# SenseTime-FVG/OpenDWM

Measured on NVIDIA H100. Metric: CTSD-3.5 6view x 16f denoise-steps/sec, higher is better.
Workload: dtype fp16

## Files before the change

### opendwm_b200/csrc/common.cuh

```cuda
#pragma once

#include <cuda.h>
#include <cuda_runtime.h>
#include <cuda_bf16.h>
#include <cuda_fp16.h>
#include <cuda_fp8.h>
#include <stdint.h>
#include <stdio.h>

namespace dwm {

void set_last_error(const char* fmt, ...);

#define DWM_CHECK_CUDA(expr)                                                   \
  do {                                                                         \
    cudaError_t _e = (expr);                                                   \
    if (_e != cudaSuccess) {                                                   \
      ::dwm::set_last_error("%s failed: %s (%s:%d)", #expr,                    \
                            cudaGetErrorString(_e), __FILE__, __LINE__);       \
      return -2;                                                               \
    }                                                                          \
  } while (0)

#define DWM_REQUIRE(cond, ...)                                                 \
  do {                                                                         \
    if (!(cond)) {                                                             \
      ::dwm::set_last_error(__VA_ARGS__);                                      \
      return -1;                                                               \
    }                                                                          \
  } while (0)

int make_tmap_2d(CUtensorMap* map, const void* base, uint64_t rows, uint64_t cols,
                 uint64_t ld, uint32_t box_rows, uint32_t box_cols, int elem_bytes);

int make_tmap_3d(CUtensorMap* map, const void* base, uint64_t items, uint64_t rows, uint64_t cols,
                 uint64_t ld, uint64_t item_ld, uint32_t box_rows, uint32_t box_cols, int elem_bytes);

int make_tmap_nd(CUtensorMap* map, const void* base, int rank, const uint64_t* dims,
                 const uint64_t* strides_bytes, const uint32_t* box, int elem_bytes);

int sm_count();

inline bool is_aligned(const void* p, uintptr_t bytes) { return (reinterpret_cast<uintptr_t>(p) & (bytes - 1)) == 0; }

#ifdef __CUDACC__
__device__ __forceinline__ uint32_t smem_u32(const void* p) {
  return static_cast<uint32_t>(__cvta_generic_to_shared(p));
}

__device__ __forceinline__ bool elect_one() {
  uint32_t pred = 0;
  asm volatile(
      "{\n\t"
      ".reg .pred P;\n\t"
      "elect.sync _|P, 0xffffffff;\n\t"
      "selp.u32 %0, 1, 0, P;\n\t"
      "}\n"
      : "=r"(pred));
  return pred != 0;
}

__device__ __forceinline__ void mbar_init(uint64_t* bar, uint32_t count) {
  asm volatile("mbarrier.init.shared::cta.b64 [%0], %1;" ::"r"(smem_u32(bar)), "r"(count));
}
__device__ __forceinline__ void fence_barrier_init() {
  asm volatile("fence.mbarrier_init.release.cluster;" ::: "memory");
}
__device__ __forceinline__ void fence_proxy_async() {
  asm volatile("fence.proxy.async.shared::cta;" ::: "memory");
}
__device__ __forceinline__ void mbar_expect_tx(uint64_t* bar, uint32_t bytes) {
  asm volatile("mbarrier.arrive.expect_tx.shared::cta.b64 _, [%0], %1;" ::"r"(smem_u32(bar)),
               "r"(bytes)
               : "memory");
}
__device__ __forceinline__ void mbar_arrive(uint64_t* bar) {
  asm volatile("mbarrier.arrive.shared::cta.b64 _, [%0];" ::"r"(smem_u32(bar)) : "memory");
}
__device__ __forceinline__ bool mbar_try_wait(uint64_t* bar, uint32_t parity) {
  uint32_t ok;
  asm volatile(
      "{\n\t"
      ".reg .pred P;\n\t"
      "mbarrier.try_wait.parity.shared::cta.b64 P, [%1], %2;\n\t"
      "selp.u32 %0, 1, 0, P;\n\t"
      "}\n"
      : "=r"(ok)
      : "r"(smem_u32(bar)), "r"(parity)
      : "memory");
  return ok != 0;
}
__device__ __forceinline__ void mbar_wait(uint64_t* bar, uint32_t parity) {
#ifdef DWM_BOUNDED_WAIT
  for (uint32_t it = 0; it < (1u << 26); ++it) {
    if (mbar_try_wait(bar, parity)) return;
  }
  printf("dwm_b200: mbarrier wait timed out (block %d thread %d)\n", blockIdx.x, threadIdx.x);
  __trap();
#else
  while (!mbar_try_wait(bar, parity)) {
  }
#endif
}

__device__ __forceinline__ void tma_prefetch_desc(const CUtensorMap* m) {
  asm volatile("prefetch.tensormap [%0];" ::"l"(reinterpret_cast<uint64_t>(m)) : "memory");
}
__device__ __forceinline__ void tma_load_2d(const CUtensorMap* m, uint64_t* bar, void* smem,
                                            int32_t c0, int32_t c1, uint64_t cache_hint) {
  asm volatile(
      "cp.async.bulk.tensor.2d.shared::cluster.global.mbarrier::complete_tx::bytes.L2::cache_hint"
      " [%0], [%1, {%3, %4}], [%2], %5;"
      :
      : "r"(smem_u32(smem)), "l"(reinterpret_cast<uint64_t>(m)), "r"(smem_u32(bar)), "r"(c0),
        "r"(c1), "l"(cache_hint)
      : "memory");
}
constexpr uint64_t kEvictNormal = 0x1000000000000000ull;
constexpr uint64_t kEvictFirst = 0x12F0000000000000ull;
constexpr uint64_t kEvictLast = 0x14F0000000000000ull;
__device__ __forceinline__ void tma_prefetch_2d(const CUtensorMap* m, int32_t c0, int32_t c1) {
  asm volatile("cp.async.bulk.prefetch.tensor.2d.L2.global.tile [%0, {%1, %2}];" ::"l"(
                   reinterpret_cast<uint64_t>(m)),
               "r"(c0), "r"(c1)
               : "memory");
}
__device__ __forceinline__ void tma_prefetch_5d(const CUtensorMap* m, int c0, int c1, int c2, int c3, int c4) {
  asm volatile("cp.async.bulk.prefetch.tensor.5d.L2.global.tile [%0, {%1, %2, %3, %4, %5}];" ::"l"(
                   reinterpret_cast<uint64_t>(m)),
               "r"(c0), "r"(c1), "r"(c2), "r"(c3), "r"(c4)
               : "memory");
}
__device__ __forceinline__ void tma_load_5d(const CUtensorMap* m, uint64_t* bar, void* smem, int c0,
                                            int c1, int c2, int c3, int c4, uint64_t hint) {
  asm volatile(
      "cp.async.bulk.tensor.5d.shared::cluster.global.mbarrier::complete_tx::bytes.L2::cache_hint"
      " [%0], [%1, {%3, %4, %5, %6, %7}], [%2], %8;"
      :
      : "r"(smem_u32(smem)), "l"(reinterpret_cast<uint64_t>(m)), "r"(smem_u32(bar)), "r"(c0), "r"(c1),
        "r"(c2), "r"(c3), "r"(c4), "l"(hint)
      : "memory");
}

__device__ __forceinline__ void tma_store_3d(const CUtensorMap* m, const void* smem, int c0, int c1, int c2) {
  asm volatile("cp.async.bulk.tensor.3d.global.shared::cta.bulk_group [%0, {%2, %3, %4}], [%1];" ::"l"(
                   reinterpret_cast<uint64_t>(m)),
               "r"(smem_u32(smem)), "r"(c0), "r"(c1), "r"(c2)
               : "memory");
}
__device__ __forceinline__ void bulk_commit() { asm volatile("cp.async.bulk.commit_group;" ::: "memory"); }
__device__ __forceinline__ void bulk_wait_read_all() { asm volatile("cp.async.bulk.wait_group.read 0;" ::: "memory"); }
__device__ __forceinline__ void bulk_wait_all() { asm volatile("cp.async.bulk.wait_group 0;" ::: "memory"); }
__device__ __forceinline__ void named_bar_sync(int id, int n) {
  asm volatile("bar.sync %0, %1;" ::"r"(id), "r"(n) : "memory");
}
__device__ __forceinline__ void stmatrix_x4(uint32_t addr, uint32_t r0, uint32_t r1, uint32_t r2, uint32_t r3) {
  asm volatile("stmatrix.sync.aligned.m8n8.x4.shared.b16 [%0], {%1, %2, %3, %4};" ::"r"(addr), "r"(r0), "r"(r1),
               "r"(r2), "r"(r3)
               : "memory");
}

__device__ __forceinline__ uint32_t cluster_ctarank() {
  uint32_t r;
  asm volatile("mov.u32 %0, %%cluster_ctarank;" : "=r"(r));
  return r;
}
__device__ __forceinline__ void cluster_sync_all() {
  asm volatile("barrier.cluster.arrive.release.aligned;" ::: "memory");
  asm volatile("barrier.cluster.wait.acquire.aligned;" ::: "memory");
}
__device__ __forceinline__ uint32_t mapa_u32(uint32_t smem_addr, uint32_t rank) {
  uint32_t r;
  asm volatile("mapa.shared::cluster.u32 %0, %1, %2;" : "=r"(r) : "r"(smem_addr), "r"(rank));
  return r;
}
__device__ __forceinline__ void mbar_arrive_remote(uint32_t cluster_addr) {
  asm volatile("mbarrier.arrive.shared::cluster.b64 _, [%0];" ::"r"(cluster_addr) : "memory");
}
__device__ __forceinline__ void tma_load_2d_mc(const CUtensorMap* m, uint64_t* bar, void* smem, int32_t c0,
                                               int32_t c1, uint16_t mask, uint64_t cache_hint) {
  asm volatile(
      "cp.async.bulk.tensor.2d.shared::cluster.global.mbarrier::complete_tx::bytes.multicast::cluster"
      ".L2::cache_hint [%0], [%1, {%3, %4}], [%2], %5, %6;"
      :
      : "r"(smem_u32(smem)), "l"(reinterpret_cast<uint64_t>(m)), "r"(smem_u32(bar)), "r"(c0), "r"(c1),
        "h"(mask), "l"(cache_hint)
      : "memory");
}

__device__ __forceinline__ uint64_t gmma_desc_sw128(uint32_t smem_addr) {
  uint64_t d = 0;
  d |= static_cast<uint64_t>((smem_addr & 0x3FFFF) >> 4);
  d |= static_cast<uint64_t>(1) << 16;
  d |= static_cast<uint64_t>(1024 >> 4) << 32;
  d |= static_cast<uint64_t>(1) << 62;
  return d;
}
__device__ __forceinline__ void wgmma_fence() { asm volatile("wgmma.fence.sync.aligned;" ::: "memory"); }
__device__ __forceinline__ void wgmma_commit() { asm volatile("wgmma.commit_group.sync.aligned;" ::: "memory"); }
template <int N>
__device__ __forceinline__ void wgmma_wait() {
  asm volatile("wgmma.wait_group.sync.aligned %0;" ::"n"(N) : "memory");
}
template <int N>
__device__ __forceinline__ void fence_operands(float (&d)[N]) {
#pragma unroll
  for (int i = 0; i < N; ++i) asm volatile("" : "+f"(d[i])::"memory");
}
template <int R>
__device__ __forceinline__ void setmaxnreg_inc() { asm volatile("setmaxnreg.inc.sync.aligned.u32 %0;" ::"n"(R)); }
template <int R>
__device__ __forceinline__ void setmaxnreg_dec() { asm volatile("setmaxnreg.dec.sync.aligned.u32 %0;" ::"n"(R)); }

__device__ __forceinline__ float gelu_erf(float x) {
  return 0.5f * x * (1.0f + erff(x * 0.70710678118654752440f));
}
__device__ __forceinline__ float gelu_tanh(float x) {
  const float k2 = 2.0f * 0.7978845608028654f;
  const float u2 = k2 * (x + 0.044715f * x * x * x);
  return __fdividef(x, 1.0f + __expf(-u2));
}
__device__ __forceinline__ float silu(float x) { return x / (1.0f + __expf(-x)); }

template <typename T>
struct Cvt;
template <>
struct Cvt<__nv_bfloat16> {
  __device__ static __forceinline__ uint32_t pack2(float a, float b) {
    __nv_bfloat162 v = __floats2bfloat162_rn(a, b);
    return *reinterpret_cast<uint32_t*>(&v);
  }
  __device__ static __forceinline__ float2 unpack2(uint32_t u) {
    __nv_bfloat162 v = *reinterpret_cast<__nv_bfloat162*>(&u);
    return __bfloat1622float2(v);
  }
  __device__ static __forceinline__ float to_f(__nv_bfloat16 v) { return __bfloat162float(v); }
  __device__ static __forceinline__ __nv_bfloat16 from_f(float v) { return __float2bfloat16_rn(v); }
};
template <>
struct Cvt<__half> {
  __device__ static __forceinline__ uint32_t pack2(float a, float b) {
    __half2 v = __floats2half2_rn(a, b);
    return *reinterpret_cast<uint32_t*>(&v);
  }
  __device__ static __forceinline__ float2 unpack2(uint32_t u) {
    __half2 v = *reinterpret_cast<__half2*>(&u);
    return __half22float2(v);
  }
  __device__ static __forceinline__ float to_f(__half v) { return __half2float(v); }
  __device__ static __forceinline__ __half from_f(float v) { return __float2half_rn(v); }
};

__device__ __forceinline__ float warp_sum(float v) {
#pragma unroll
  for (int o = 16; o > 0; o >>= 1) v += __shfl_xor_sync(0xffffffffu, v, o);
  return v;
}
__device__ __forceinline__ float warp_max(float v) {
#pragma unroll
  for (int o = 16; o > 0; o >>= 1) v = fmaxf(v, __shfl_xor_sync(0xffffffffu, v, o));
  return v;
}

constexpr float kE4M3Max = 448.f;
__device__ __forceinline__ float e4m3_inv(float amax) { return amax > 0.f ? __fdiv_rn(kE4M3Max, amax) : 0.f; }
__device__ __forceinline__ float e4m3_scale(float amax) { return amax > 0.f ? __fdiv_rn(amax, kE4M3Max) : 1.f; }
__device__ __forceinline__ uint32_t e4m3x4(float a, float b, float c, float d, float inv) {
  uint16_t lo, hi;
  asm("cvt.rn.satfinite.e4m3x2.f32 %0, %1, %2;" : "=h"(lo) : "f"(__fmul_rn(b, inv)), "f"(__fmul_rn(a, inv)));
  asm("cvt.rn.satfinite.e4m3x2.f32 %0, %1, %2;" : "=h"(hi) : "f"(__fmul_rn(d, inv)), "f"(__fmul_rn(c, inv)));
  return static_cast<uint32_t>(lo) | (static_cast<uint32_t>(hi) << 16);
}
#endif

}
```

### opendwm_b200/csrc/gemm.cu

```cuda
#include <stdlib.h>
#include <string.h>

#include "gemm_epilogue.cuh"

namespace dwm {

constexpr int STAGES = 4;
constexpr int A_STAGE_BYTES = BM * BK * 2;

static_assert(EPI_BOXES_BYTES >= EPI_STAGE_BYTES, "epilogue region");
template <int NT>
struct GemmCfg {
  static constexpr int kBStageBytes = NT * BK * 2;
  static constexpr int kSmemBytes =
      STAGES * (A_STAGE_BYTES + kBStageBytes) + EPI_BOXES_BYTES + 1024  + 256 ;
};

template <typename TA, typename T, int EPI, int NT, int CL>
__global__ void __launch_bounds__(GEMM_THREADS, 1)
    gemm_wgmma_kernel(const __grid_constant__ CUtensorMap tmap_a,
                      const __grid_constant__ CUtensorMap tmap_b,
                      const __grid_constant__ CUtensorMap tmap_out, int M, int N, int K,
                      EpiParams p) {
  constexpr int B_STAGE_BYTES = GemmCfg<NT>::kBStageBytes;
  constexpr int BKE = BK * 2 / static_cast<int>(sizeof(TA));
  extern __shared__ uint8_t smem_raw[];
  uint8_t* smem = smem_raw + ((1024u - (smem_u32(smem_raw) & 1023u)) & 1023u);
  uint8_t* smem_a = smem;
  uint8_t* smem_b = smem + STAGES * A_STAGE_BYTES;
  uint8_t* epi_region = smem + STAGES * (A_STAGE_BYTES + B_STAGE_BYTES);
  float* epi_stage = reinterpret_cast<float*>(epi_region);
  uint64_t* bars = reinterpret_cast<uint64_t*>(epi_region + EPI_BOXES_BYTES);
  uint64_t* full_bar = bars;
  uint64_t* empty_bar = bars + STAGES;

  const int warp = threadIdx.x >> 5;
  const int lane = threadIdx.x & 31;
  const int wg = threadIdx.x >> 7;
  const uint32_t rank = CL == 2 ? cluster_ctarank() : 0u;

  const int m_blocks = (M + BM - 1) / BM;
  const int n_blocks = (N + NT - 1) / NT;
  const int k_blocks = (K + BKE - 1) / BKE;
  const int num_tiles = ((m_blocks + CL - 1) / CL) * n_blocks;
  const int first = static_cast<int>(blockIdx.x) / CL, step = static_cast<int>(gridDim.x) / CL;

  if (warp == 0 && lane == 0) {
    tma_prefetch_desc(&tmap_a);
    tma_prefetch_desc(&tmap_b);
    for (int s = 0; s < STAGES; ++s) {
      mbar_init(&full_bar[s], 1);
      mbar_init(&empty_bar[s], CL * EPI_WARPS);
    }
    fence_barrier_init();
  }
  if constexpr (CL == 2) cluster_sync_all(); else __syncthreads();

  if (wg == 0) {
    setmaxnreg_dec<PRODUCER_REGS>();
    if (warp == 0 && elect_one()) {
      int stage = 0;
      uint32_t phase = 0;
      for (int tile = first; tile < num_tiles; tile += step) {
        const int m_blk = (tile / n_blocks) * CL + static_cast<int>(rank);
        const int n_blk = tile % n_blocks;
        for (int kb = 0; kb < k_blocks; ++kb) {
          mbar_wait(&empty_bar[stage], phase ^ 1);
          mbar_expect_tx(&full_bar[stage], A_STAGE_BYTES + B_STAGE_BYTES);
          tma_load_2d(&tmap_a, &full_bar[stage], smem_a + stage * A_STAGE_BYTES, kb * BKE,
                      m_blk * BM, kEvictNormal);
          if constexpr (CL == 2) {
            tma_load_2d_mc(&tmap_b, &full_bar[stage], smem_b + stage * B_STAGE_BYTES + rank * (B_STAGE_BYTES / 2),
                           kb * BKE, n_blk * NT + static_cast<int>(rank) * (NT / 2), 0x3, kEvictLast);
          } else {
            tma_load_2d(&tmap_b, &full_bar[stage], smem_b + stage * B_STAGE_BYTES, kb * BKE,
                        n_blk * NT, kEvictLast);
          }
          if (++stage == STAGES) {
            stage = 0;
            phase ^= 1;
          }
        }
      }
    }
    __syncwarp();
  } else {
    setmaxnreg_inc<CONSUMER_REGS>();
    const int cw = wg - 1;
    const int wrow = cw * 64 + (warp & 3) * 16;
    float* stg = epi_stage + (warp - 4) * 512;
    TmaOut tout{epi_out16(EPI) && p.tma_out, &tmap_out, epi_region + cw * 2 * EPI_BOX_BYTES, 1 + cw,
                (threadIdx.x & 127) == 0, 0};
    int stage = 0;
    uint32_t phase = 0;
    for (int tile = first; tile < num_tiles; tile += step) {
      const int m_blk = (tile / n_blocks) * CL + static_cast<int>(rank);
      const int n_blk = tile % n_blocks;
      const int t = threadIdx.x & 127;
      prefetch_resid_tile<EPI, NT>(p, m_blk * BM + cw * 64 + (t >> 1), M, n_blk * NT, N, t & 1);
      float acc[NT / 2];
      wg_mainloop<TA, NT, CL>(acc, smem_a, A_STAGE_BYTES, cw * 64 * 128, smem_b, B_STAGE_BYTES, full_bar,
                              empty_bar, STAGES, k_blocks, stage, phase, lane, rank ^ 1u);
      if constexpr (sizeof(TA) == 1)
        dequant_frag<NT>(acc, p.a_scale, p.w_scale, m_blk * BM + wrow, M, n_blk * NT, N, lane);
      drain_tile<T, EPI, NT>(acc, stg, m_blk * BM, wrow, M, n_blk * NT, N, p, lane, TileGeom{0, 0, 0, 0, 0}, &tout);
    }
    if (tout.on && tout.leader) bulk_wait_all();
  }
  if constexpr (CL == 2) cluster_sync_all();
}

int g_resid_tma = 1;

template <typename TA, typename T, int EPI, int NT, int CL>
static int launch_gemm(const dwm_linear_args* a, cudaStream_t stream) {
  constexpr int eb = static_cast<int>(sizeof(TA));
  CUtensorMap ta, tb;
  int rc = make_tmap_2d(&ta, a->A, a->M, a->K, a->lda, BM, BK * 2 / eb, eb);
  if (rc) return rc;
  rc = make_tmap_2d(&tb, a->W, a->N, a->K, a->ldw, NT / CL, BK * 2 / eb, eb);
  if (rc) return rc;

  EpiParams p;
  fill_epi_params(p, a);
  p.resid_prefetch = g_resid_tma;
  CUtensorMap to = {};
  if (epi_out16(EPI) && a->n_peer_out == 0) {
    const long long rpi = a->rows_per_item > 0 ? a->rows_per_item : a->M;
    const long long items = a->M / rpi;
    const long long item_ld = (a->rows_per_item > 0 ? a->out_item_stride : a->M) * a->ldo;
    const long long n_out = (EPI == DWM_EPI_GEGLU || EPI == DWM_EPI_GEGLU_TANH) ? a->N / 2 : a->N;
    if (items > 0) {
      rc = make_tmap_3d(&to, reinterpret_cast<const T*>(a->out) + a->out_row_offset * a->ldo, items, rpi, n_out,
                        a->ldo, item_ld, 64, 64, 2);
      if (rc) return rc;
    }
    p.tma_out = 1;
    p.out_rpi = static_cast<int>(rpi);
    p.out_items = static_cast<int>(items);
  }

  constexpr int smem_bytes = GemmCfg<NT>::kSmemBytes;
  auto kern = gemm_wgmma_kernel<TA, T, EPI, NT, CL>;
  static bool attr_set = false;
  if (!attr_set) {
    DWM_CHECK_CUDA(cudaFuncSetAttribute(kern, cudaFuncAttributeMaxDynamicSharedMemorySize, smem_bytes));
    attr_set = true;
  }
  const long long m_blocks = (a->M + BM - 1) / BM;
  const long long n_blocks = (a->N + NT - 1) / NT;
  const long long tiles = ((m_blocks + CL - 1) / CL) * n_blocks;
  const long long slots = sm_count() / CL;
  const int grid = CL * static_cast<int>(tiles < slots ? tiles : slots);
  const int Mi = static_cast<int>(a->M), Ni = static_cast<int>(a->N), Ki = static_cast<int>(a->K);
  if constexpr (CL == 1) {
    kern<<<grid, GEMM_THREADS, smem_bytes, stream>>>(ta, tb, to, Mi, Ni, Ki, p);
  } else {
    DWM_CHECK_CUDA(launch_cluster2(kern, grid, GEMM_THREADS, smem_bytes, stream,
                                   ta, tb, to, Mi, Ni, Ki, p));
  }
  DWM_CHECK_CUDA(cudaGetLastError());
  return 0;
}

int g_gemm_bn = 0;
int g_gemm_2cta = -1;

static int pick_tile_n(const dwm_linear_args* a, int cl) {
  if (a->epilogue == DWM_EPI_GEGLU || a->epilogue == DWM_EPI_GEGLU_TANH) return 256;
  if (g_gemm_bn == 128 || g_gemm_bn == 256) return g_gemm_bn;
  const long long slots = sm_count() / cl;
  const long long m_groups = ((a->M + BM - 1) / BM + cl - 1) / cl;
  const long long t256 = m_groups * ((a->N + 255) / 256), t128 = m_groups * ((a->N + 127) / 128);
  const long long waves256 = (t256 + slots - 1) / slots, waves128 = (t128 + slots - 1) / slots;
  return waves128 * 128 * 10 < waves256 * 256 * 9 ? 128 : 256;
}

template <typename TA, typename T, int EPI, int CL>
static int launch_pick_n(const dwm_linear_args* a, cudaStream_t s) {
  if (pick_tile_n(a, CL) == 128) return launch_gemm<TA, T, EPI, 128, CL>(a, s);
  return launch_gemm<TA, T, EPI, 256, CL>(a, s);
}

template <typename TA, typename T, int CL, typename TF = T>
static int dispatch_epi(const dwm_linear_args* a, cudaStream_t s) {
  if constexpr (sizeof(TA) == 2) {
    if (a->epilogue == DWM_EPI_STORE && a->act == DWM_ACT_QUICK_GELU)
      return launch_pick_n<TA, T, EPI_STORE_QUICK_GELU, CL>(a, s);
    if (a->epilogue == DWM_EPI_GEGLU_TANH) return launch_gemm<TA, T, DWM_EPI_GEGLU_TANH, 256, CL>(a, s);
  }
  switch (a->epilogue) {
    case DWM_EPI_STORE: return launch_pick_n<TA, T, DWM_EPI_STORE, CL>(a, s);
    case DWM_EPI_GEGLU: return launch_gemm<TA, T, DWM_EPI_GEGLU, 256, CL>(a, s);
    case DWM_EPI_QKNORM: return launch_pick_n<TA, T, DWM_EPI_QKNORM, CL>(a, s);
    case DWM_EPI_RESID: return launch_pick_n<TA, TF, DWM_EPI_RESID, CL>(a, s);
    case DWM_EPI_F32: return launch_pick_n<TA, TF, DWM_EPI_F32, CL>(a, s);
    default: set_last_error("dwm_b200_linear: unknown epilogue %d", a->epilogue); return -1;
  }
}

template <int CL>
static int dispatch_e4m3(const dwm_linear_args* a, cudaStream_t s) {
  if (a->out_dtype == DWM_BF16) return dispatch_epi<__nv_fp8_e4m3, __nv_bfloat16, CL>(a, s);
  return dispatch_epi<__nv_fp8_e4m3, __half, CL, __nv_bfloat16>(a, s);
}

}

namespace dwm { int g_attn_tc = -1; extern int g_ln_staged; extern int g_conv_2cta; extern int g_conv_halo; }

extern "C" int dwm_b200_set_option(const char* name, int value) {
  using namespace dwm;
  DWM_REQUIRE(name != nullptr, "dwm_b200_set_option: null name");
  if (strcmp(name, "attn_tc") == 0) { g_attn_tc = value; return 0; }
  if (strcmp(name, "ln_staged") == 0) { g_ln_staged = value; return 0; }
  if (strcmp(name, "gemm_bn") == 0) { g_gemm_bn = value; return 0; }
  if (strcmp(name, "gemm_2cta") == 0) { g_gemm_2cta = value; return 0; }
  if (strcmp(name, "resid_tma") == 0) { g_resid_tma = value; return 0; }
  if (strcmp(name, "conv_2cta") == 0) { g_conv_2cta = value; return 0; }
  if (strcmp(name, "conv_halo") == 0) { g_conv_halo = value; return 0; }
  set_last_error("dwm_b200_set_option: unknown option %s", name);
  return -1;
}

extern "C" int dwm_b200_linear(const dwm_linear_args* a, dwm_stream_t stream) {
  using namespace dwm;
  DWM_REQUIRE(a != nullptr, "dwm_b200_linear: null args");
  DWM_REQUIRE(a->M > 0 && a->N > 0 && a->K > 0, "dwm_b200_linear: empty problem %lld x %lld x %lld",
              (long long)a->M, (long long)a->N, (long long)a->K);
  DWM_REQUIRE(a->M < (1ll << 31) && a->N < (1ll << 31) && a->K < (1ll << 31),
              "dwm_b200_linear: dimension exceeds int32");
  DWM_REQUIRE(a->A && a->W && a->out, "dwm_b200_linear: null A/W/out");
  DWM_REQUIRE(a->K % 8 == 0 && a->lda % 8 == 0 && a->ldw % 8 == 0,
              "dwm_b200_linear: K, lda, ldw must be multiples of 8 (16-byte TMA pitch); got %lld %lld %lld",
              (long long)a->K, (long long)a->lda, (long long)a->ldw);
  if (a->dtype == DWM_E4M3) {
    DWM_REQUIRE(a->K % 16 == 0 && a->lda % 16 == 0 && a->ldw % 16 == 0,
                "dwm_b200_linear: E4M3 needs K, lda, ldw multiples of 16 (16-byte TMA pitch); got %lld %lld %lld",
                (long long)a->K, (long long)a->lda, (long long)a->ldw);
    DWM_REQUIRE(a->a_scale && a->w_scale, "dwm_b200_linear: E4M3 operands need a_scale and w_scale");
    DWM_REQUIRE(a->out_dtype == DWM_BF16 || a->out_dtype == DWM_F16,
                "dwm_b200_linear: E4M3 operands need out_dtype DWM_BF16 or DWM_F16, got %d", a->out_dtype);
    DWM_REQUIRE((reinterpret_cast<uintptr_t>(a->w_scale) & 7) == 0,
                "dwm_b200_linear: w_scale must be 8-byte aligned");
  }
  DWM_REQUIRE((reinterpret_cast<uintptr_t>(a->A) & 15) == 0 &&
                  (reinterpret_cast<uintptr_t>(a->W) & 15) == 0 &&
                  (reinterpret_cast<uintptr_t>(a->out) & 15) == 0,
              "dwm_b200_linear: A, W, out must be 16-byte aligned");
  DWM_REQUIRE(a->N % 32 == 0, "dwm_b200_linear: N must be a multiple of 32, got %lld", (long long)a->N);
  DWM_REQUIRE(a->ldo % 8 == 0, "dwm_b200_linear: ldo must be a multiple of 8");
  if (a->epilogue == DWM_EPI_GEGLU || a->epilogue == DWM_EPI_GEGLU_TANH)
    DWM_REQUIRE(a->N % 256 == 0, "dwm_b200_linear: GEGLU needs N %% 256 == 0 (packed weight)");
  if (a->epilogue == DWM_EPI_GEGLU_TANH || a->act == DWM_ACT_QUICK_GELU) {
    DWM_REQUIRE(a->dtype == DWM_BF16 || a->dtype == DWM_F16,
                "dwm_b200_linear: DWM_EPI_GEGLU_TANH and DWM_ACT_QUICK_GELU need 16-bit operands");
    DWM_REQUIRE(a->act != DWM_ACT_QUICK_GELU || a->epilogue == DWM_EPI_STORE,
                "dwm_b200_linear: DWM_ACT_QUICK_GELU needs the DWM_EPI_STORE epilogue");
  }
  if (a->epilogue == DWM_EPI_QKNORM) {
    DWM_REQUIRE(a->N % 64 == 0 && a->qk_region > 0 && a->qk_region % 64 == 0 && a->q_norm_weight &&
                    (a->k_norm_weight || a->qk_norm_regions == 1),
                "dwm_b200_linear: QKNORM needs head_dim 64 regions and both norm weights");
  }
  DWM_REQUIRE(a->n_peer_out >= 0 && a->n_peer_out <= 8, "dwm_b200_linear: n_peer_out out of range");
  if (a->n_peer_out > 0)
    DWM_REQUIRE(a->epilogue == DWM_EPI_STORE || a->epilogue == DWM_EPI_QKNORM || a->epilogue == DWM_EPI_GEGLU ||
                    a->epilogue == DWM_EPI_GEGLU_TANH,
                "dwm_b200_linear: peer_out needs a 16-bit epilogue");
  if (a->epilogue == DWM_EPI_RESID && a->blend_x)
    DWM_REQUIRE(a->alpha != nullptr, "dwm_b200_linear: blend_x without alpha");
  for (const void* p : {static_cast<const void*>(a->bias), static_cast<const void*>(a->resid),
                        static_cast<const void*>(a->gate), static_cast<const void*>(a->blend_x)})
    DWM_REQUIRE((reinterpret_cast<uintptr_t>(p) & 15) == 0,
                "dwm_b200_linear: bias, resid, gate, blend_x must be 16-byte aligned");
  for (int i = 0; i < a->n_peer_out; ++i)
    DWM_REQUIRE(a->peer_out[i] && (reinterpret_cast<uintptr_t>(a->peer_out[i]) & 15) == 0,
                "dwm_b200_linear: peer_out[%d] must be a 16-byte aligned pointer", i);
  DWM_REQUIRE((!a->resid || a->ldr % 4 == 0) && (!a->gate || a->gate_ld % 4 == 0) &&
                  (!a->blend_x || a->ldx % 4 == 0),
              "dwm_b200_linear: ldr, gate_ld, ldx must be multiples of 4 (16-byte rows); got %lld %lld %lld",
              (long long)a->ldr, (long long)a->gate_ld, (long long)a->ldx);
  if (a->rows_per_item > 0 && a->epilogue != DWM_EPI_RESID && a->epilogue != DWM_EPI_F32)
    DWM_REQUIRE(a->out_item_stride >= a->rows_per_item,
                "dwm_b200_linear: out_item_stride %lld < rows_per_item %lld would write several items "
                "to the same output rows", (long long)a->out_item_stride, (long long)a->rows_per_item);
  cudaStream_t s = reinterpret_cast<cudaStream_t>(stream);
  if (g_gemm_2cta < 0) {
    const char* e = getenv("DWM_GEMM_2CTA");
    g_gemm_2cta = (e && e[0] == '0') ? 0 : 1;
  }
  const bool pair = g_gemm_2cta == 1 && a->M >= 512;
  if (a->dtype == DWM_BF16)
    return pair ? dispatch_epi<__nv_bfloat16, __nv_bfloat16, 2>(a, s) : dispatch_epi<__nv_bfloat16, __nv_bfloat16, 1>(a, s);
  if (a->dtype == DWM_F16) return pair ? dispatch_epi<__half, __half, 2>(a, s) : dispatch_epi<__half, __half, 1>(a, s);
  if (a->dtype == DWM_E4M3) return pair ? dispatch_e4m3<2>(a, s) : dispatch_e4m3<1>(a, s);
  set_last_error("dwm_b200_linear: dtype must be DWM_BF16, DWM_F16 or DWM_E4M3, got %d", a->dtype);
  return -1;
}
```

### opendwm_b200/csrc/gemm_epilogue.cuh

```cuda
#pragma once
#include "common.cuh"
#include "wgmma.cuh"
#include "../../include/dwm_b200.h"

namespace dwm {

constexpr int BM = 128;
constexpr int BK = 64;
constexpr int WG_K = 16;
constexpr int CONSUMER_WGS = 2;
constexpr int GEMM_THREADS = 128 * (1 + CONSUMER_WGS);
constexpr int EPI_WARPS = 4 * CONSUMER_WGS;
constexpr int EPI_STAGE_BYTES = EPI_WARPS * 16 * 32 * 4;
constexpr int EPI_BOX_BYTES = 64 * 64 * 2;
constexpr int EPI_BOXES_BYTES = CONSUMER_WGS * 2 * EPI_BOX_BYTES;
constexpr int PRODUCER_REGS = 40;
constexpr int CONSUMER_REGS = 232;
constexpr int EPI_STORE_QUICK_GELU = 16;

__host__ __device__ constexpr bool epi_out16(int epi) {
  return epi == DWM_EPI_STORE || epi == DWM_EPI_GEGLU || epi == DWM_EPI_QKNORM || epi == EPI_STORE_QUICK_GELU ||
         epi == DWM_EPI_GEGLU_TANH;
}

__device__ __forceinline__ float quick_gelu(float x) { return x / (1.0f + __expf(-1.702f * x)); }

struct EpiParams {
  void* out;
  long long ldo;
  const float* bias;
  int act;
  long long rows_per_item, out_item_stride, out_row_offset;
  const float* qw;
  const float* kw;
  long long qk_region;
  float eps;
  int norm_regions;
  const float* resid;
  long long ldr, resid_row_mod;
  const float* gate;
  long long gate_ld;
  const float* blend_x;
  long long ldx;
  const float* alpha;
  long long rows_per_batch;
  void* peer_out[8];
  int n_peers;
  int resid_prefetch;
  const float* a_scale;
  const float* w_scale;
  int tma_out;
  int out_rpi, out_items;
};

struct TmaOut {
  bool on;
  const CUtensorMap* map;
  uint8_t* bufs;
  int bar;
  bool leader;
  uint32_t boxes;
};

__device__ __forceinline__ float apply_act(float v, int act) {
  switch (act) {
    case DWM_ACT_GELU_TANH: return gelu_tanh(v);
    case DWM_ACT_GELU_ERF: return gelu_erf(v);
    case DWM_ACT_SILU: return silu(v);
    case DWM_ACT_RELU: return fmaxf(v, 0.f);
    default: return v;
  }
}

__device__ __forceinline__ float resid_elem(float acc, float b, float g, float r) {
  return __fmaf_rn(__fadd_rn(acc, b), g, r);
}
__device__ __forceinline__ float blend_elem(float a, float a1, float x, float v) {
  return __fmaf_rn(a, x, __fmul_rn(a1, v));
}

__device__ __forceinline__ void st_global_v4(void* p, uint32_t a, uint32_t b, uint32_t c,
                                             uint32_t d) {
  asm volatile("st.global.v4.b32 [%0], {%1, %2, %3, %4};" ::"l"(p), "r"(a), "r"(b), "r"(c), "r"(d)
               : "memory");
}


template <int NA>
__device__ __forceinline__ void frag_chunk(const float (&acc)[NA], int c, float (&v)[16]) {
#pragma unroll
  for (int i = 0; i < 16; ++i) v[i] = acc[16 * c + i];
}

__device__ __forceinline__ void stage_dump(float* stg, int lane, const float (&v)[16]) {
  __syncwarp();
  const int r0 = lane >> 2, q0 = (lane & 3) >> 1, h = (lane & 1) * 2;
#pragma unroll
  for (int jj = 0; jj < 4; ++jj) {
    const int q = (2 * jj + q0) ^ r0;
    *reinterpret_cast<float2*>(stg + r0 * 32 + q * 4 + h) = make_float2(v[4 * jj], v[4 * jj + 1]);
    *reinterpret_cast<float2*>(stg + (r0 + 8) * 32 + q * 4 + h) = make_float2(v[4 * jj + 2], v[4 * jj + 3]);
  }
  __syncwarp();
}

__device__ __forceinline__ int frag_col(int lane, int jj, int e) { return 8 * jj + 2 * (lane & 3) + (e & 1); }

struct TileGeom {
  int bw;
  int rows;
  int w_lim;
  int h_lim;
  int img_w;
};

template <typename T, int EPI, int NT>
__device__ __forceinline__ void drain_tile(const float (&acc)[NT / 2], float* stg, int m_base, int row0, int M,
                                           int n_tile0, int N, const EpiParams& p, int lane,
                                           const TileGeom geom = TileGeom{0, 0, 0, 0, 0}, TmaOut* tma = nullptr) {
  constexpr bool kOut16 = epi_out16(EPI);
  const bool use_tma = kOut16 && tma != nullptr && tma->on;
  const int rs = lane >> 3;
  const int c4 = lane & 7;

  int orow[4];
  int rrow[4];
  int item[4];
  float alpha[4];
  const int rpi = static_cast<int>(p.rows_per_item);
#pragma unroll
  for (int it = 0; it < 4 && !use_tma; ++it) {
    int m;
    bool valid;
    if (geom.bw > 0) {
      const int r = row0 + it * 4 + rs;
      const int ph = r / geom.bw, pw = r - ph * geom.bw;
      valid = r < geom.rows && pw < geom.w_lim && ph < geom.h_lim;
      m = m_base + ph * geom.img_w + pw;
    } else {
      m = m_base + row0 + it * 4 + rs;
      valid = m < M;
    }
    if (valid) {
      int o = m;
      if (kOut16) {
        if (rpi > 0) o = (m / rpi) * static_cast<int>(p.out_item_stride) + (m % rpi);
        o += static_cast<int>(p.out_row_offset);
      }
      orow[it] = o;
      if (EPI == DWM_EPI_RESID) {
        item[it] = rpi > 0 ? m / rpi : 0;
        rrow[it] = p.resid_row_mod > 0 ? m % static_cast<int>(p.resid_row_mod)
                   : (p.resid_row_mod < 0 ? item[it] : m);
        alpha[it] = p.blend_x ? __ldg(p.alpha + (p.rows_per_batch > 0 ? m / static_cast<int>(p.rows_per_batch) : 0)) : 0.f;
      }
    } else {
      orow[it] = -1;
    }
  }

  auto stg4 = [&](int r) { return *reinterpret_cast<const float4*>(stg + r * 32 + ((c4 ^ (r & 7)) << 2)); };
  auto flush16 = [&](int ocol) {
#pragma unroll
    for (int it = 0; it < 4; ++it) {
      const float4 v = stg4(it * 4 + rs);
      if (orow[it] >= 0) {
        T* dst = reinterpret_cast<T*>(p.out) + static_cast<long long>(orow[it]) * p.ldo + ocol + c4 * 4;
        uint2 pk;
        pk.x = Cvt<T>::pack2(v.x, v.y);
        pk.y = Cvt<T>::pack2(v.z, v.w);
        *reinterpret_cast<uint2*>(dst) = pk;
        const long long eoff = static_cast<long long>(orow[it]) * p.ldo + ocol + c4 * 4;
        for (int q = 0; q < p.n_peers; ++q)
          *reinterpret_cast<uint2*>(reinterpret_cast<T*>(p.peer_out[q]) + eoff) = pk;
      }
    }
  };
  auto box_put = [&](const float (&v)[16], int ocol) {
    const uint32_t buf = smem_u32(tma->bufs + (tma->boxes & 1) * EPI_BOX_BYTES);
    const int i = lane >> 3;
    const int r = (row0 & 63) + (i & 1) * 8 + (lane & 7);
#pragma unroll
    for (int q = 0; q < 2; ++q) {
      const int c16 = ((ocol >> 5) & 1) * 4 + 2 * q + (i >> 1);
      stmatrix_x4(buf + r * 128 + ((c16 ^ (r & 7)) << 4), Cvt<T>::pack2(v[8 * q], v[8 * q + 1]),
                  Cvt<T>::pack2(v[8 * q + 2], v[8 * q + 3]), Cvt<T>::pack2(v[8 * q + 4], v[8 * q + 5]),
                  Cvt<T>::pack2(v[8 * q + 6], v[8 * q + 7]));
    }
  };
  auto box_store = [&](int ocol) {
    fence_proxy_async();
    if (tma->leader) bulk_wait_read_all();
    named_bar_sync(tma->bar, 128);
    const uint8_t* buf = tma->bufs + (tma->boxes & 1) * EPI_BOX_BYTES;
    const int m0 = m_base + (row0 & ~63), col = ocol & ~63;
    const int item = m0 / p.out_rpi, r = m0 - item * p.out_rpi;
    if (tma->leader) {
      if (item < p.out_items) tma_store_3d(tma->map, buf, col, r, item);
      bulk_commit();
    }
    const int j0 = item < p.out_items ? p.out_rpi - r : 0;
    const int j1 = M - m0 < 64 ? M - m0 : 64;
    if (j0 < j1) {
      const int t = ((row0 & 63) << 1) + lane;
      const int c = t & 7;
      const int n_out = (EPI == DWM_EPI_GEGLU || EPI == DWM_EPI_GEGLU_TANH) ? N / 2 : N;
#pragma unroll 1
      for (int j = j0 + (t >> 3); j < j1; j += 16) {
        const int m = m0 + j;
        if (col + 8 * c < n_out) {
          const long long o = static_cast<long long>(m / p.out_rpi) * p.out_item_stride + m % p.out_rpi + p.out_row_offset;
          *reinterpret_cast<uint4*>(reinterpret_cast<T*>(p.out) + o * p.ldo + col + 8 * c) =
              *reinterpret_cast<const uint4*>(buf + j * 128 + ((c ^ (j & 7)) << 4));
        }
      }
    }
    ++tma->boxes;
  };
  auto put16 = [&](const float (&v)[16], int ocol, bool box_done) {
    if (use_tma) {
      box_put(v, ocol);
      if (box_done) box_store(ocol);
    } else {
      stage_dump(stg, lane, v);
      flush16(ocol);
    }
  };
  float4 rq[4], bq[4];
  auto prefetch32 = [&](int ocol) {
    if constexpr (EPI == DWM_EPI_RESID) {
      const int col = ocol + c4 * 4;
#pragma unroll
      for (int it = 0; it < 4; ++it) {
        rq[it] = make_float4(0.f, 0.f, 0.f, 0.f);
        bq[it] = make_float4(0.f, 0.f, 0.f, 0.f);
        if (orow[it] >= 0) {
          if (p.resid) rq[it] = *reinterpret_cast<const float4*>(p.resid + static_cast<long long>(rrow[it]) * p.ldr + col);
          if (p.blend_x) bq[it] = *reinterpret_cast<const float4*>(p.blend_x + static_cast<long long>(orow[it]) * p.ldx + col);
        }
      }
    }
  };
  auto flush32 = [&](int ocol) {
    const int col = ocol + c4 * 4;
    float4 b = make_float4(0.f, 0.f, 0.f, 0.f);
    if (EPI == DWM_EPI_RESID && p.bias) b = __ldg(reinterpret_cast<const float4*>(p.bias + col));
#pragma unroll
    for (int it = 0; it < 4; ++it) {
      float4 v = stg4(it * 4 + rs);
      if (orow[it] >= 0) {
        if (EPI == DWM_EPI_RESID) {
          float4 g = make_float4(1.f, 1.f, 1.f, 1.f);
          if (p.gate)
            g = __ldg(reinterpret_cast<const float4*>(p.gate + static_cast<long long>(item[it]) * p.gate_ld + col));
          v.x = resid_elem(v.x, b.x, g.x, rq[it].x); v.y = resid_elem(v.y, b.y, g.y, rq[it].y);
          v.z = resid_elem(v.z, b.z, g.z, rq[it].z); v.w = resid_elem(v.w, b.w, g.w, rq[it].w);
          if (p.blend_x) {
            const float a = alpha[it], a1 = 1.0f - alpha[it];
            v.x = blend_elem(a, a1, bq[it].x, v.x); v.y = blend_elem(a, a1, bq[it].y, v.y);
            v.z = blend_elem(a, a1, bq[it].z, v.z); v.w = blend_elem(a, a1, bq[it].w, v.w);
          }
        }
        *reinterpret_cast<float4*>(reinterpret_cast<float*>(p.out) + static_cast<long long>(orow[it]) * p.ldo + col) = v;
      }
    }
  };

  if constexpr (EPI == DWM_EPI_STORE || EPI == DWM_EPI_F32 || EPI == DWM_EPI_RESID || EPI == EPI_STORE_QUICK_GELU) {
#pragma unroll
    for (int c = 0; c < NT / 32; ++c) {
      const int n0 = n_tile0 + c * 32;
      if (n0 >= N) break;
      prefetch32(n0);
      float v[16];
      frag_chunk(acc, c, v);
      if (EPI != DWM_EPI_RESID) {
        if (p.bias) {
#pragma unroll
          for (int jj = 0; jj < 4; ++jj) {
            const float2 b = __ldg(reinterpret_cast<const float2*>(p.bias + n0 + frag_col(lane, jj, 0)));
            v[4 * jj] += b.x; v[4 * jj + 1] += b.y; v[4 * jj + 2] += b.x; v[4 * jj + 3] += b.y;
          }
        }
        if constexpr (EPI == EPI_STORE_QUICK_GELU) {
#pragma unroll
          for (int j = 0; j < 16; ++j) v[j] = quick_gelu(v[j]);
        } else if (p.act == DWM_ACT_GELU_TANH) {
#pragma unroll
          for (int j = 0; j < 16; ++j) v[j] = gelu_tanh(v[j]);
        } else if (p.act == DWM_ACT_SILU) {
#pragma unroll
          for (int j = 0; j < 16; ++j) v[j] = silu(v[j]);
        } else if (p.act == DWM_ACT_GELU_ERF) {
#pragma unroll
          for (int j = 0; j < 16; ++j) v[j] = gelu_erf(v[j]);
        } else if (p.act == DWM_ACT_RELU) {
#pragma unroll
          for (int j = 0; j < 16; ++j) v[j] = fmaxf(v[j], 0.f);
        }
      }
      if constexpr (kOut16) {
        put16(v, n0, c & 1);
      } else {
        stage_dump(stg, lane, v);
        flush32(n0);
      }
    }
    if (use_tma && N - n_tile0 < NT && ((N - n_tile0) & 32)) box_store(N - 32);
  } else if constexpr (EPI == DWM_EPI_GEGLU || EPI == DWM_EPI_GEGLU_TANH) {
    static_assert(NT == 256, "GEGLU packs value / gate halves per 256-column tile");
#pragma unroll
    for (int c = 0; c < 4; ++c) {
      float a[16], g[16], v[16];
      frag_chunk(acc, c, a);
      frag_chunk(acc, c + 4, g);
      const float* bv = p.bias ? p.bias + n_tile0 + c * 32 : nullptr;
#pragma unroll
      for (int j = 0; j < 16; ++j) {
        float x = a[j], y = g[j];
        if (bv) {
          const int col = frag_col(lane, j >> 2, j);
          x += __ldg(bv + col);
          y += __ldg(bv + 128 + col);
        }
        v[j] = x * (EPI == DWM_EPI_GEGLU ? gelu_erf(y) : gelu_tanh(y));
      }
      put16(v, n_tile0 / 2 + c * 32, c & 1);
    }
  } else {
#pragma unroll
    for (int g = 0; g < NT / 64; ++g) {
      const int n0 = n_tile0 + g * 64;
      if (n0 >= N) break;
      float v0[16], v1[16];
      frag_chunk(acc, 2 * g, v0);
      frag_chunk(acc, 2 * g + 1, v1);
      if (p.bias) {
#pragma unroll
        for (int j = 0; j < 16; ++j) {
          const int col = frag_col(lane, j >> 2, j);
          v0[j] += __ldg(p.bias + n0 + col);
          v1[j] += __ldg(p.bias + n0 + 32 + col);
        }
      }
      const int region = n0 / static_cast<int>(p.qk_region);
      if (region < p.norm_regions) {
        const float* w = region == 0 ? p.qw : p.kw;
        float ss_lo = 0.f, ss_hi = 0.f;
#pragma unroll
        for (int j = 0; j < 16; ++j) {
          if ((j & 3) < 2) ss_lo += v0[j] * v0[j] + v1[j] * v1[j];
          else ss_hi += v0[j] * v0[j] + v1[j] * v1[j];
        }
        ss_lo += __shfl_xor_sync(0xffffffffu, ss_lo, 1);
        ss_lo += __shfl_xor_sync(0xffffffffu, ss_lo, 2);
        ss_hi += __shfl_xor_sync(0xffffffffu, ss_hi, 1);
        ss_hi += __shfl_xor_sync(0xffffffffu, ss_hi, 2);
        const float inv_lo = rsqrtf(ss_lo * (1.0f / 64.0f) + p.eps);
        const float inv_hi = rsqrtf(ss_hi * (1.0f / 64.0f) + p.eps);
#pragma unroll
        for (int j = 0; j < 16; ++j) {
          const int col = frag_col(lane, j >> 2, j);
          const float inv = (j & 3) < 2 ? inv_lo : inv_hi;
          v0[j] = v0[j] * inv * __ldg(w + col);
          v1[j] = v1[j] * inv * __ldg(w + 32 + col);
        }
      }
      put16(v0, n0, false);
      put16(v1, n0 + 32, true);
    }
  }
}

template <int NT>
__device__ __forceinline__ void dequant_frag(float (&acc)[NT / 2], const float* a_scale, const float* w_scale,
                                             int m0, int M, int n_tile0, int N, int lane) {
  const int r = m0 + (lane >> 2);
  const float s_lo = r < M ? __ldg(a_scale + r) : 0.f;
  const float s_hi = r + 8 < M ? __ldg(a_scale + r + 8) : 0.f;
#pragma unroll
  for (int g = 0; g < NT / 64; ++g) {
    float2 w[8];
#pragma unroll
    for (int jj = 0; jj < 8; ++jj) {
      const int col = n_tile0 + 8 * (8 * g + jj) + 2 * (lane & 3);
      w[jj] = col < N ? __ldg(reinterpret_cast<const float2*>(w_scale + col)) : make_float2(0.f, 0.f);
    }
#pragma unroll
    for (int jj = 0; jj < 8; ++jj) {
      const int j = 8 * g + jj;
      acc[4 * j + 0] = __fmul_rn(acc[4 * j + 0], __fmul_rn(s_lo, w[jj].x));
      acc[4 * j + 1] = __fmul_rn(acc[4 * j + 1], __fmul_rn(s_lo, w[jj].y));
      acc[4 * j + 2] = __fmul_rn(acc[4 * j + 2], __fmul_rn(s_hi, w[jj].x));
      acc[4 * j + 3] = __fmul_rn(acc[4 * j + 3], __fmul_rn(s_hi, w[jj].y));
    }
    asm volatile("" ::: "memory");
  }
}

template <int NT>
__device__ __forceinline__ void dequant_frag_vol(float (&acc)[NT / 2], float s, const float* w_scale,
                                                 int n_tile0, int N, int lane) {
#pragma unroll
  for (int g = 0; g < NT / 32; ++g) {
    constexpr int G = 4;
    float2 w[G];
#pragma unroll
    for (int jj = 0; jj < G; ++jj) {
      const int col = n_tile0 + 8 * (G * g + jj) + 2 * (lane & 3);
      w[jj] = col < N ? __ldg(reinterpret_cast<const float2*>(w_scale + col)) : make_float2(0.f, 0.f);
    }
#pragma unroll
    for (int jj = 0; jj < G; ++jj) {
      const int j = G * g + jj;
      const float sx = __fmul_rn(s, w[jj].x), sy = __fmul_rn(s, w[jj].y);
      acc[4 * j + 0] = __fmul_rn(acc[4 * j + 0], sx);
      acc[4 * j + 1] = __fmul_rn(acc[4 * j + 1], sy);
      acc[4 * j + 2] = __fmul_rn(acc[4 * j + 2], sx);
      acc[4 * j + 3] = __fmul_rn(acc[4 * j + 3], sy);
    }
    asm volatile("" ::: "memory");
  }
}

template <typename T, int NT, int CL = 1, int TAPS = 1>
__device__ __forceinline__ void wg_mainloop(float (&acc)[NT / 2], const uint8_t* smem_a, int a_stage_bytes,
                                            int a_row_off_bytes, const uint8_t* smem_b, int b_stage_bytes,
                                            uint64_t* full_bar, uint64_t* empty_bar, int stages, int k_iters,
                                            int& stage, uint32_t& phase, int lane, uint32_t peer = 0) {
#pragma unroll
  for (int i = 0; i < NT / 2; ++i) acc[i] = 0.f;
  fence_operands(acc);
  auto release = [&](int s) {
    mbar_arrive(&empty_bar[s]);
    if constexpr (CL == 2) mbar_arrive_remote(mapa_u32(smem_u32(&empty_bar[s]), peer));
  };
  int prev = -1;
  for (int ki = 0; ki < k_iters; ++ki) {
    mbar_wait(&full_bar[stage], phase);
    wgmma_fence();
#pragma unroll
    for (int t = 0; t < TAPS; ++t) {
      const uint64_t da = gmma_desc_sw128(smem_u32(smem_a + stage * a_stage_bytes + a_row_off_bytes + t * 128));
      const uint64_t db = gmma_desc_sw128(smem_u32(smem_b + stage * b_stage_bytes + t * NT * BK * 2));
#pragma unroll
      for (int k = 0; k < BK / WG_K; ++k) Wgmma<NT, T>::ss(acc, da + 2 * k, db + 2 * k, 1u);
    }
    wgmma_commit();
    wgmma_wait<1>();
    if (prev >= 0 && lane == 0) release(prev);
    prev = stage;
    if (++stage == stages) { stage = 0; phase ^= 1; }
  }
  wgmma_wait<0>();
  fence_operands(acc);
  if (prev >= 0 && lane == 0) release(prev);
}

template <int EPI, int NT>
__device__ __forceinline__ void prefetch_resid_tile(const EpiParams& p, int m, int M, int n_tile0,
                                                    int N, int half) {
  constexpr int half_cols = NT / 2;
  if constexpr (EPI == DWM_EPI_RESID) {
    if (!p.resid_prefetch) return;
    const int n0 = n_tile0 + half * half_cols;
    if (m < M && n0 < N) {
      const int cols = (N - n0) < half_cols ? (N - n0) : half_cols;
      const uint32_t bytes = static_cast<uint32_t>(cols) * 4u;
      if (p.resid) {
        if (p.resid_row_mod >= 0) {
          const long long rr = p.resid_row_mod > 0 ? m % static_cast<int>(p.resid_row_mod) : m;
          const float* src = p.resid + rr * p.ldr + n0;
          asm volatile("cp.async.bulk.prefetch.L2.global [%0], %1;" ::"l"(src), "r"(bytes) : "memory");
        }
      }
      if (p.blend_x) {
        const float* src = p.blend_x + static_cast<long long>(m) * p.ldx + n0;
        asm volatile("cp.async.bulk.prefetch.L2.global [%0], %1;" ::"l"(src), "r"(bytes) : "memory");
      }
    }
  }
}

template <typename... KArgs, typename... Args>
inline cudaError_t launch_cluster2(void (*kern)(KArgs...), int grid, int threads, int smem, cudaStream_t s,
                                   Args... args) {
  cudaLaunchConfig_t cfg = {};
  cfg.gridDim = dim3(grid);
  cfg.blockDim = dim3(threads);
  cfg.dynamicSmemBytes = smem;
  cfg.stream = s;
  cudaLaunchAttribute attr[1];
  attr[0].id = cudaLaunchAttributeClusterDimension;
  attr[0].val.clusterDim.x = 2;
  attr[0].val.clusterDim.y = 1;
  attr[0].val.clusterDim.z = 1;
  cfg.attrs = attr;
  cfg.numAttrs = 1;
  return cudaLaunchKernelEx(&cfg, kern, args...);
}

inline void fill_epi_params(EpiParams& p, const dwm_linear_args* a) {
  p.out = a->out;
  p.ldo = a->ldo;
  p.bias = a->bias;
  p.act = a->act;
  p.rows_per_item = a->rows_per_item;
  p.out_item_stride = a->out_item_stride;
  p.out_row_offset = a->out_row_offset;
  p.qw = a->q_norm_weight;
  p.kw = a->k_norm_weight;
  p.qk_region = a->qk_region;
  p.eps = a->eps;
  p.norm_regions = a->qk_norm_regions > 0 ? a->qk_norm_regions : 2;
  p.resid = a->resid;
  p.ldr = a->ldr;
  p.resid_row_mod = a->resid_row_mod;
  p.gate = a->gate;
  p.gate_ld = a->gate_ld;
  p.blend_x = a->blend_x;
  p.ldx = a->ldx;
  p.alpha = a->alpha;
  p.rows_per_batch = a->rows_per_batch;
  p.n_peers = a->n_peer_out;
  p.resid_prefetch = 1;
  for (int i = 0; i < 8; ++i) p.peer_out[i] = i < a->n_peer_out ? a->peer_out[i] : nullptr;
  p.a_scale = a->a_scale;
  p.w_scale = a->w_scale;
  p.tma_out = 0;
  p.out_rpi = p.out_items = 0;
}

}
```

Baseline: 1.210.

## Use TMA for fp32 GEMM epilogue stores and residual loads

Extends the TMA-based epilogue to fp32 outputs (F32 and RESID epilogues). Residual tiles are loaded by TMA into double-buffered shared-memory boxes, gated by new mbarriers, then combined with the accumulator and written back with 2D TMA stores. This replaces per-thread global loads and stores and the prefetch path for these cases. It adds synchronization, extra barrier state and more shared-memory traffic per box, and it is restricted to residual cases without row modulo or blend.

After: 1.223 (median of 6 runs). 1.01x the previous value.

```diff
diff --git a/opendwm_b200/csrc/common.cuh b/opendwm_b200/csrc/common.cuh
--- a/opendwm_b200/csrc/common.cuh
+++ b/opendwm_b200/csrc/common.cuh
@@ -148,6 +148,13 @@
                "r"(smem_u32(smem)), "r"(c0), "r"(c1), "r"(c2)
                : "memory");
 }
+__device__ __forceinline__ void tma_store_2d(const CUtensorMap* m, const void* smem, int c0, int c1,
+                                             uint64_t cache_hint) {
+  asm volatile("cp.async.bulk.tensor.2d.global.shared::cta.bulk_group.L2::cache_hint [%0, {%2, %3}], [%1], %4;" ::"l"(
+                   reinterpret_cast<uint64_t>(m)),
+               "r"(smem_u32(smem)), "r"(c0), "r"(c1), "l"(cache_hint)
+               : "memory");
+}
 __device__ __forceinline__ void bulk_commit() { asm volatile("cp.async.bulk.commit_group;" ::: "memory"); }
 __device__ __forceinline__ void bulk_wait_read_all() { asm volatile("cp.async.bulk.wait_group.read 0;" ::: "memory"); }
 __device__ __forceinline__ void bulk_wait_all() { asm volatile("cp.async.bulk.wait_group 0;" ::: "memory"); }
diff --git a/opendwm_b200/csrc/gemm.cu b/opendwm_b200/csrc/gemm.cu
--- a/opendwm_b200/csrc/gemm.cu
+++ b/opendwm_b200/csrc/gemm.cu
@@ -20,7 +20,8 @@
 __global__ void __launch_bounds__(GEMM_THREADS, 1)
     gemm_wgmma_kernel(const __grid_constant__ CUtensorMap tmap_a,
                       const __grid_constant__ CUtensorMap tmap_b,
-                      const __grid_constant__ CUtensorMap tmap_out, int M, int N, int K,
+                      const __grid_constant__ CUtensorMap tmap_out,
+                      const __grid_constant__ CUtensorMap tmap_resid, int M, int N, int K,
                       EpiParams p) {
   constexpr int B_STAGE_BYTES = GemmCfg<NT>::kBStageBytes;
   constexpr int BKE = BK * 2 / static_cast<int>(sizeof(TA));
@@ -33,6 +34,7 @@
   uint64_t* bars = reinterpret_cast<uint64_t*>(epi_region + EPI_BOXES_BYTES);
   uint64_t* full_bar = bars;
   uint64_t* empty_bar = bars + STAGES;
+  uint64_t* resid_bar = bars + 2 * STAGES;
 
   const int warp = threadIdx.x >> 5;
   const int lane = threadIdx.x & 31;
@@ -52,6 +54,7 @@
       mbar_init(&full_bar[s], 1);
       mbar_init(&empty_bar[s], CL * EPI_WARPS);
     }
+    for (int i = 0; i < CONSUMER_WGS * 2; ++i) mbar_init(&resid_bar[i], 1);
     fence_barrier_init();
   }
   if constexpr (CL == 2) cluster_sync_all(); else __syncthreads();
@@ -89,8 +92,8 @@
     const int cw = wg - 1;
     const int wrow = cw * 64 + (warp & 3) * 16;
     float* stg = epi_stage + (warp - 4) * 512;
-    TmaOut tout{epi_out16(EPI) && p.tma_out, &tmap_out, epi_region + cw * 2 * EPI_BOX_BYTES, 1 + cw,
-                (threadIdx.x & 127) == 0, 0};
+    TmaOut tout{p.tma_out != 0, &tmap_out, epi_region + cw * 2 * EPI_BOX_BYTES, 1 + cw,
+                (threadIdx.x & 127) == 0, 0, &tmap_resid, resid_bar + cw * 2, 0};
     int stage = 0;
     uint32_t phase = 0;
     for (int tile = first; tile < num_tiles; tile += step) {
@@ -98,6 +101,7 @@
       const int n_blk = tile % n_blocks;
       const int t = threadIdx.x & 127;
       prefetch_resid_tile<EPI, NT>(p, m_blk * BM + cw * 64 + (t >> 1), M, n_blk * NT, N, t & 1);
+      tma_resid_prologue<EPI>(tout, m_blk * BM + cw * 64, n_blk * NT, N);
       float acc[NT / 2];
       wg_mainloop<TA, NT, CL>(acc, smem_a, A_STAGE_BYTES, cw * 64 * 128, smem_b, B_STAGE_BYTES, full_bar,
                               empty_bar, STAGES, k_blocks, stage, phase, lane, rank ^ 1u);
@@ -124,7 +128,7 @@
   EpiParams p;
   fill_epi_params(p, a);
   p.resid_prefetch = g_resid_tma;
-  CUtensorMap to = {};
+  CUtensorMap to = {}, tr = {};
   if (epi_out16(EPI) && a->n_peer_out == 0) {
     const long long rpi = a->rows_per_item > 0 ? a->rows_per_item : a->M;
     const long long items = a->M / rpi;
@@ -139,6 +143,15 @@
     p.out_rpi = static_cast<int>(rpi);
     p.out_items = static_cast<int>(items);
   }
+  if (!epi_out16(EPI) && (EPI == DWM_EPI_F32 || (a->resid && a->resid_row_mod == 0 && !a->blend_x))) {
+    rc = make_tmap_2d(&to, a->out, a->M, a->N, a->ldo, 64, 32, 4);
+    if (rc) return rc;
+    if (EPI == DWM_EPI_RESID) {
+      rc = make_tmap_2d(&tr, a->resid, a->M, a->N, a->ldr, 64, 32, 4);
+      if (rc) return rc;
+    }
+    p.tma_out = 1;
+  }
 
   constexpr int smem_bytes = GemmCfg<NT>::kSmemBytes;
   auto kern = gemm_wgmma_kernel<TA, T, EPI, NT, CL>;
@@ -154,10 +167,10 @@
   const int grid = CL * static_cast<int>(tiles < slots ? tiles : slots);
   const int Mi = static_cast<int>(a->M), Ni = static_cast<int>(a->N), Ki = static_cast<int>(a->K);
   if constexpr (CL == 1) {
-    kern<<<grid, GEMM_THREADS, smem_bytes, stream>>>(ta, tb, to, Mi, Ni, Ki, p);
+    kern<<<grid, GEMM_THREADS, smem_bytes, stream>>>(ta, tb, to, tr, Mi, Ni, Ki, p);
   } else {
     DWM_CHECK_CUDA(launch_cluster2(kern, grid, GEMM_THREADS, smem_bytes, stream,
-                                   ta, tb, to, Mi, Ni, Ki, p));
+                                   ta, tb, to, tr, Mi, Ni, Ki, p));
   }
   DWM_CHECK_CUDA(cudaGetLastError());
   return 0;
diff --git a/opendwm_b200/csrc/gemm_epilogue.cuh b/opendwm_b200/csrc/gemm_epilogue.cuh
--- a/opendwm_b200/csrc/gemm_epilogue.cuh
+++ b/opendwm_b200/csrc/gemm_epilogue.cuh
@@ -60,7 +60,24 @@
   int bar;
   bool leader;
   uint32_t boxes;
+  const CUtensorMap* resid_map;
+  uint64_t* rbars;
+  uint32_t rphase;
 };
+
+__device__ __forceinline__ void tma_resid_load(TmaOut& t, uint32_t box, int col, int m0) {
+  const uint32_t b = box & 1;
+  mbar_expect_tx(&t.rbars[b], EPI_BOX_BYTES);
+  tma_load_2d(t.resid_map, &t.rbars[b], t.bufs + b * EPI_BOX_BYTES, col, m0, kEvictFirst);
+}
+template <int EPI>
+__device__ __forceinline__ void tma_resid_prologue(TmaOut& t, int m0, int n_tile0, int N) {
+  if constexpr (EPI == DWM_EPI_RESID) {
+    if (!t.on || !t.leader) return;
+    bulk_wait_read_all();
+    for (int c = 0; c < 2 && n_tile0 + 32 * c < N; ++c) tma_resid_load(t, t.boxes + c, n_tile0 + 32 * c, m0);
+  }
+}
 
 __device__ __forceinline__ float apply_act(float v, int act) {
   switch (act) {
@@ -119,7 +136,7 @@
                                            int n_tile0, int N, const EpiParams& p, int lane,
                                            const TileGeom geom = TileGeom{0, 0, 0, 0, 0}, TmaOut* tma = nullptr) {
   constexpr bool kOut16 = epi_out16(EPI);
-  const bool use_tma = kOut16 && tma != nullptr && tma->on;
+  const bool use_tma = tma != nullptr && tma->on;
   const int rs = lane >> 3;
   const int c4 = lane & 7;
 
@@ -213,6 +230,57 @@
           *reinterpret_cast<uint4*>(reinterpret_cast<T*>(p.out) + o * p.ldo + col + 8 * c) =
               *reinterpret_cast<const uint4*>(buf + j * 128 + ((c ^ (j & 7)) << 4));
         }
+      }
+    }
+    ++tma->boxes;
+  };
+  auto put32 = [&](const float (&v)[16], int c, int ocol) {
+    const uint32_t b = tma->boxes & 1;
+    uint8_t* buf = tma->bufs + b * EPI_BOX_BYTES;
+    const int m0 = m_base + (row0 & ~63);
+    float2 bb[4], g[2][4];
+    if constexpr (EPI == DWM_EPI_RESID) {
+#pragma unroll
+      for (int jj = 0; jj < 4; ++jj)
+        bb[jj] = p.bias ? __ldg(reinterpret_cast<const float2*>(p.bias + ocol + frag_col(lane, jj, 0)))
+                        : make_float2(0.f, 0.f);
+#pragma unroll
+      for (int h = 0; h < 2; ++h) {
+        const int m = m0 + (row0 & 63) + (lane >> 2) + 8 * h;
+        const float* gp = p.gate && m < M
+                              ? p.gate + static_cast<long long>(rpi > 0 ? m / rpi : 0) * p.gate_ld + ocol : nullptr;
+#pragma unroll
+        for (int jj = 0; jj < 4; ++jj)
+          g[h][jj] = gp ? __ldg(reinterpret_cast<const float2*>(gp + frag_col(lane, jj, 0))) : make_float2(1.f, 1.f);
+      }
+      mbar_wait(&tma->rbars[b], (tma->rphase >> b) & 1);
+      tma->rphase ^= 1u << b;
+    }
+#pragma unroll
+    for (int h = 0; h < 2; ++h) {
+      const int r = (row0 & 63) + (lane >> 2) + 8 * h;
+#pragma unroll
+      for (int jj = 0; jj < 4; ++jj) {
+        float2* q = reinterpret_cast<float2*>(buf + r * 128 + (((2 * jj + ((lane & 3) >> 1)) ^ (r & 7)) << 4) +
+                                              (lane & 1) * 8);
+        float2 x = make_float2(v[4 * jj + 2 * h], v[4 * jj + 2 * h + 1]);
+        if constexpr (EPI == DWM_EPI_RESID) {
+          const float2 rr = *q;
+          x.x = resid_elem(x.x, bb[jj].x, g[h][jj].x, rr.x);
+          x.y = resid_elem(x.y, bb[jj].y, g[h][jj].y, rr.y);
+        }
+        *q = x;
+      }
+    }
+    fence_proxy_async();
+    if (EPI != DWM_EPI_RESID && tma->leader) bulk_wait_read_all();
+    named_bar_sync(tma->bar, 128);
+    if (tma->leader) {
+      tma_store_2d(tma->map, buf, ocol, m0, kEvictFirst);
+      bulk_commit();
+      if (EPI == DWM_EPI_RESID && c + 2 < NT / 32 && ocol + 64 < N) {
+        bulk_wait_read_all();
+        tma_resid_load(*tma, tma->boxes + 2, ocol + 64, m0);
       }
     }
     ++tma->boxes;
@@ -271,7 +339,7 @@
     for (int c = 0; c < NT / 32; ++c) {
       const int n0 = n_tile0 + c * 32;
       if (n0 >= N) break;
-      prefetch32(n0);
+      if (!use_tma) prefetch32(n0);
       float v[16];
       frag_chunk(acc, c, v);
       if (EPI != DWM_EPI_RESID) {
@@ -301,12 +369,15 @@
       }
       if constexpr (kOut16) {
         put16(v, n0, c & 1);
+      } else if (use_tma) {
+        put32(v, c, n0);
       } else {
         stage_dump(stg, lane, v);
         flush32(n0);
       }
     }
-    if (use_tma && N - n_tile0 < NT && ((N - n_tile0) & 32)) box_store(N - 32);
+    if constexpr (kOut16)
+      if (use_tma && N - n_tile0 < NT && ((N - n_tile0) & 32)) box_store(N - 32);
   } else if constexpr (EPI == DWM_EPI_GEGLU || EPI == DWM_EPI_GEGLU_TANH) {
     static_assert(NT == 256, "GEGLU packs value / gate halves per 256-column tile");
 #pragma unroll
```
